# OpenNLPLab/ACR_WSSS

Measured on AMD Instinct MI355X. Metric: img/s ACR-ViT-hybrid-base 448x448 train step, higher is better.
Workload: dtype f32_split; 1 GPU; BASELINE configs[1]: ViT-hybrid-base (DPT) 448x448, batch 16 per GPU, ACR train step (2 views, fwd+bwd+SGD); global_batch=16, classes=20, alpha=125, parallelism=dp1

## Files before the change

### acr_wsss_amd/csrc/attn_f32.h

```cpp
#pragma once
#include <hip/hip_runtime.h>
#include <stdint.h>

struct AttnGeom {
    int B, H, T;
    float scale;
    int64_t sb, st, sh;
    int64_t osb, ost, osh;
};

void acr_attn_fwd_f32_dma(const AttnGeom& g, const float* q, const float* k, const float* v, float* o, float* lse2, float* pmean,
                          int64_t pmean_sb, int64_t pmean_st, hipStream_t st);
void acr_attn_bwd_f32_dma(const AttnGeom& g, const float* q, const float* k, const float* v, const float* o, const float* d_o,
                          const float* lse2, const float* gm, int64_t gm_sb, int64_t gm_st, float* dq, float* dk, float* dv,
                          float* delta, hipStream_t st);

void acr_attn_fwd_f32_sres(const AttnGeom& g, const float* q, const float* k, const float* v, float* o, float* lse2, float* scores,
                           float* pmean, int64_t pmean_sb, int64_t pmean_st, hipStream_t st);
void acr_attn_bwd_f32_sres(const AttnGeom& g, const float* q, const float* k, const float* v, const float* o, const float* d_o,
                           const float* lse2, const float* scores, const float* gm, int64_t gm_sb, int64_t gm_st, float* dq,
                           float* dk, float* dv, float* delta, hipStream_t st);
void acr_attn_pmean_sres(const AttnGeom& g, const float* scores, const float* lse2, float* pmean, int64_t pmean_sb, int64_t pmean_st,
                         hipStream_t st);
void acr_attn_delta_sres(const AttnGeom& g, const float* scores, const float* o, const float* d_o, const float* lse2, const float* gm,
                         int64_t gm_sb, int64_t gm_st, float* delta, hipStream_t st);

int64_t acr_attn_x3_scores_floats(const AttnGeom& g);
int64_t acr_attn_x3_bwd_ws_floats(const AttnGeom& g);
bool acr_attn_x3_fwd_uses_split_tail(int T);
void acr_attn_fwd_f32_x3(const AttnGeom& g, const float* q, const float* k, const float* v, float* o, float* lse2, float* scores,
                         float* pmean, int64_t pmean_sb, int64_t pmean_st, hipStream_t st, char* oimg = nullptr);
void acr_attn_bwd_f32_x3(const AttnGeom& g, const float* q, const float* k, const float* v, const float* o, const float* d_o,
                         const float* lse2, const float* scores, const float* gm, int64_t gm_sb, int64_t gm_st, float* dq, float* dk,
                         float* dv, float* delta_ws, hipStream_t st);
```

### acr_wsss_amd/csrc/attn_f32_sres.hip

```cpp
#include <type_traits>

#include "acr_common.h"
#include "attn_f32.h"
#include "attn_f32_tiles.h"
#include "attn_f32_scores.h"
#include "attn_f32_sres_tails.h"


template <int NW>
__global__ __launch_bounds__(64 * NW, NW == 4 ? 2 : 1) void attn_fwd_sres_kernel(AttnGeom g, const float* __restrict__ q, const float* __restrict__ k,
                                                               const float* __restrict__ v, float* __restrict__ o,
                                                               float* __restrict__ lse2, float* __restrict__ sres, int ntail) {
    __shared__ __attribute__((aligned(1024))) float smem[4 * DT_FLOATS];
    __shared__ float mlsh[4 * 64];
    const int nmain = (int)gridDim.x - ntail;
    if (NW == 4 && (int)blockIdx.x >= nmain) {
        attn_fwd_tail_body<4>(smem, mlsh, g, q, k, v, o, lse2, sres, acr_xcd_remap((int)blockIdx.x - nmain, ntail));
        return;
    }
    const int NB = (g.T + 31) >> 5, nqt = ntail ? NB / NW : (NB + NW - 1) / NW;
    int id = acr_xcd_remap(blockIdx.x, nmain);
    const int qt = id % nqt; id /= nqt;
    const int hd = id % g.H;
    const int b = id / g.H;
// ... 38 lines not shown
        ATTN_SOFTMAX_STEP(s, m, l, o0, o1, p);
        __builtin_amdgcn_s_setprio(0);
        accop_x<VOFF, 0, false>(o0, p, lb);
        accop_x<VOFF, 1, false>(o1, p, lb);
    };
    for (int k0 = 0; k0 < g.T; k0 += 64) {
        step(k0, std::integral_constant<int, 0>{});
        if (k0 + 32 < g.T) step(k0 + 32, std::integral_constant<int, 1>{});
    }
    if (live && q0 + r < g.T) {
        const float inv = 1.f / l;
        ATTN_FWD_FINISH(g, o, lse2, b, hd, q0, r, h, o0, o1, m, l, inv);
    }
}

#ifndef DELTA4_MINB
#define DELTA4_MINB 1
#endif
template <int NW> __global__ __launch_bounds__(64 * NW, DELTA4_MINB) void attn_delta_sres4_kernel(AttnGeom g, int NB, const float* __restrict__ sres,
                                                               const float* __restrict__ o, const float* __restrict__ d_o,
                                                               const float* __restrict__ lse2, const float* __restrict__ gm,
                                                               int64_t gm_sb, int64_t gm_st, float* __restrict__ delta) {
    __shared__ __attribute__((aligned(16))) float gt[3][32 * 36];
    const int tid = threadIdx.x, lane = tid & 63, wave = tid >> 6;
    const int theta = lane & 31, hh = lane >> 5;
    const int HG = g.H / NW;
    const int hd = (blockIdx.x % HG) * NW + wave;
    const int t = blockIdx.x / HG;
    const int qb = t % NB, b = t / NB;
    const int qrow = qb * 32 + theta;
    const bool qok = qrow < g.T;
    const int qc = min(qrow, g.T - 1);
    float part = 0.f;
    {
        const int64_t off = (int64_t)b * g.osb + (int64_t)hd * g.osh + (int64_t)qc * g.ost + 32 * hh;
        const float* op = o + off;
        const float* dp = d_o + off;
#pragma unroll
        for (int i = 0; i < 8; ++i) {
            const f32x4 a = *reinterpret_cast<const f32x4*>(op + 4 * i), c = *reinterpret_cast<const f32x4*>(dp + 4 * i);
            part += a[0] * c[0] + a[1] * c[1] + a[2] * c[2] + a[3] * c[3];
        }
    }
    part += __shfl_xor(part, 32);
    const float l2q = qok ? lse2[((int64_t)b * g.H + hd) * g.T + qrow] : INFINITY;
    const float* sp = sres + attn_score_block(g.H, NB, b, hd, qb, 0) + lane * 4;
    const bool loader = tid < 256;
    const int lrow = (tid & 255) >> 3, lc = (tid & 7) * 4;
    const float* gl = gm + (int64_t)b * gm_sb + (int64_t)min(qb * 32 + lrow, g.T - 1) * gm_st + lc;
    const int nfull = g.T >> 5;
    float rho = 0.f;
    f32x4 sv[3][4], gn[3];
    auto fetch = [&](int kb, int set) {
        if (loader) gn[set] = *reinterpret_cast<const f32x4*>(gl + kb * 32);
#pragma unroll
        for (int gq = 0; gq < 4; ++gq) sv[set][gq] = SRES_LOAD_NT(sp + (int64_t)kb * SB_FLOATS + gq * 256);
// ... 89 lines not shown
        float* ob = out + (int64_t)b * out_sb;
        if (key < g.T) {
#pragma unroll
            for (int i = 0; i < 16; ++i) {
                const int row = 2 * i + hh;
                const int qq = qb * 32 + row;
                if (qq < g.T) ob[(int64_t)qq * out_st + key] = tl[row * 33 + theta];
            }
        }
    }
}

__global__ __launch_bounds__(256) void attn_delta_sres_kernel(AttnGeom g, int NB, const float* __restrict__ sres,
                                                              const float* __restrict__ o, const float* __restrict__ d_o,
                                                              const float* __restrict__ lse2, const float* __restrict__ gm,
                                                              int64_t gm_sb, int64_t gm_st, float* __restrict__ delta) {
    const int tid = threadIdx.x, lane = tid & 63, wave = tid >> 6;
    const int theta = lane & 31, hh = lane >> 5;
    int id = blockIdx.x * 4 + wave;
    if (id >= g.B * NB * g.H) return;
    const int hd = id % g.H;
    const int t = id / g.H;
    const int qb = t % NB, b = t / NB;
    const int qrow = qb * 32 + theta;
    const bool qok = qrow < g.T;
    const int qc = min(qrow, g.T - 1);
    float part = 0.f;
    {
        const int64_t off = (int64_t)b * g.osb + (int64_t)hd * g.osh + (int64_t)qc * g.ost + 32 * hh;
        const float* op = o + off;
        const float* dp = d_o + off;
#pragma unroll
        for (int i = 0; i < 8; ++i) {
            const f32x4 a = *reinterpret_cast<const f32x4*>(op + 4 * i), c = *reinterpret_cast<const f32x4*>(dp + 4 * i);
            part += a[0] * c[0] + a[1] * c[1] + a[2] * c[2] + a[3] * c[3];
        }
    }
    part += __shfl_xor(part, 32);
    float rho = 0.f;
    if (gm != nullptr) {
        const float l2q = qok ? lse2[((int64_t)b * g.H + hd) * g.T + qrow] : INFINITY;
        const float* sp = sres + attn_score_block(g.H, NB, b, hd, qb, 0) + lane * 4;
        const float* gr = gm + (int64_t)b * gm_sb + (int64_t)qc * gm_st;
        const int nfull = g.T >> 5;
#pragma unroll 4
        for (int kb = 0; kb < nfull; ++kb) {
            f32x4 sv[4], gv[4];
#pragma unroll
            for (int gq = 0; gq < 4; ++gq) {
                sv[gq] = SRES_LOAD(sp + (int64_t)kb * SB_FLOATS + gq * 256);
// ... 233 lines not shown
    const int NB = (g.T + 31) / 32;
    const int ntail = attn_split_tail(NB, 4) ? g.B * g.H : 0;
    const int nmain = g.B * g.H * (ntail ? NB / 4 : (NB + 3) / 4);
    hipLaunchKernelGGL(attn_fwd_sres_kernel<4>, dim3(nmain + ntail), dim3(256), 0, st, g, q, k, v, o, lse2, scores, ntail);
    if (pmean) acr_attn_pmean_sres(g, scores, lse2, pmean, pmean_sb, pmean_st, st);
}

void acr_attn_pmean_sres(const AttnGeom& g, const float* scores, const float* lse2, float* pmean, int64_t pmean_sb, int64_t pmean_st,
                         hipStream_t st) {
    const int NB = (g.T + 31) / 32;
    hipLaunchKernelGGL(attn_pmean_sres_kernel, dim3((g.B * NB * NB + 3) / 4), dim3(256), 0, st, g, NB, scores, lse2, pmean, pmean_sb,
                       pmean_st);
}

void acr_attn_delta_sres(const AttnGeom& g, const float* scores, const float* o, const float* d_o, const float* lse2, const float* gm,
                         int64_t gm_sb, int64_t gm_st, float* delta, hipStream_t st) {
    const int NB = (g.T + 31) / 32;
#ifndef DELTA4_NW
#define DELTA4_NW 4
#endif
    if (gm != nullptr && (g.H % DELTA4_NW) == 0 && acr_opt(ACR_OPT_ATTN_DELTA_1HEAD) == 0)
        hipLaunchKernelGGL(attn_delta_sres4_kernel<DELTA4_NW>, dim3(g.B * NB * (g.H / DELTA4_NW)), dim3(64 * DELTA4_NW), 0, st, g, NB, scores, o, d_o,
                           lse2, gm, gm_sb, gm_st, delta);
    else
        hipLaunchKernelGGL(attn_delta_sres_kernel, dim3((g.B * NB * g.H + 3) / 4), dim3(256), 0, st, g, NB, scores, o, d_o, lse2, gm, gm_sb,
                           gm_st, delta);
}

void acr_attn_bwd_f32_sres(const AttnGeom& g, const float* q, const float* k, const float* v, const float* o, const float* d_o,
                           const float* lse2, const float* scores, const float* gm, int64_t gm_sb, int64_t gm_st, float* dq,
                           float* dk, float* dv, float* delta, hipStream_t st) {
    const int nt = (g.T + 127) / 128, NB = (g.T + 31) / 32;
    acr_attn_delta_sres(g, scores, o, d_o, lse2, gm, gm_sb, gm_st, delta, st);
    const int ntail = attn_split_tail(NB, 4) ? g.B * g.H : 0;
    const int nmain = g.B * g.H * (ntail ? NB / 4 : nt);
    hipLaunchKernelGGL(attn_bwd_sres_kernel, dim3(2 * nmain + 2 * ntail), dim3(256), 0, st, g, q, k, v, d_o, lse2, (const float*)delta,
                       scores, gm, gm_sb, gm_st, dq, dk, dv, ntail);
}
```

### acr_wsss_amd/csrc/attn_f32_x3.hip

```cpp
#include <type_traits>

#include "acr_split.h"
#include "attn_f32.h"
#include "attn_f32_scores.h"
#include "attn_f32_sres_tails.h"

typedef __bf16 bf16_t;

#define X3_PLANE_B (32 * 64 * 2)
#define X3_TILE_B (3 * X3_PLANE_B)
#define X3_SLOT_B (2 * X3_TILE_B)


__device__ __forceinline__ void x3_wait_vm(int n) { attn_wait_vm<false, 9, 8, 7, 5, 4, 1>(n); }
__device__ __forceinline__ void x3_barrier(int n_younger) {
    x3_wait_vm(n_younger);
    acr_barrier_nofence();
}

struct X3Geom {
    int B, H, T, D;
    float scale;
    int64_t plane;
    int64_t osb, ost, osh;
// ... 528 lines not shown
    const int64_t n8 = (int64_t)g.B * g.T * g.H * 8;
    hipLaunchKernelGGL(x3_split_kernel, dim3((unsigned)((n8 + 255) / 256), 3), dim3(256), 0, st, a);
    const int NB = (g.T + 31) / 32;
    const int ntail = (acr_attn_x3_fwd_uses_split_tail(g.T) && oimg == nullptr) ? g.B * g.H : 0;
    hipLaunchKernelGGL(attn_fwd_x3_kernel, dim3(g.B * g.H * (ntail ? NB / 4 : (NB + 3) / 4) + ntail), dim3(256), 0, st, x, (const bf16_t*)planes,
                       (const bf16_t*)(planes + 3 * x.plane), (const bf16_t*)(planes + 6 * x.plane), o, lse2, scores, q, k, v, g, ntail, oimg);
    if (pmean) acr_attn_pmean_sres(g, scores, lse2, pmean, pmean_sb, pmean_st, st);
}

void acr_attn_bwd_f32_x3(const AttnGeom& g, const float* q, const float* k, const float* v, const float* o, const float* d_o,
                         const float* lse2, const float* scores, const float* gm, int64_t gm_sb, int64_t gm_st, float* dq, float* dk,
                         float* dv, float* delta_ws, hipStream_t st) {
    const X3Geom x = x3_geom(g);
    const bf16_t* planes = reinterpret_cast<const bf16_t*>(scores + attn_score_floats(g.B, g.H, g.T));
    bf16_t* dop = reinterpret_cast<bf16_t*>(delta_ws + (((int64_t)g.B * g.H * g.T + 3) & ~(int64_t)3));
    X3SplitArgs a;
    a.src[0] = d_o; a.src[1] = a.src[2] = nullptr;
    a.sb = g.osb; a.st = g.ost; a.sh = g.osh; a.dst = dop; a.plane = x.plane; a.B = g.B; a.T = g.T; a.H = g.H;
    const int64_t n8 = (int64_t)g.B * g.T * g.H * 8;
    hipLaunchKernelGGL(x3_split_kernel, dim3((unsigned)((n8 + 255) / 256), 1), dim3(256), 0, st, a);
    acr_attn_delta_sres(g, scores, o, d_o, lse2, gm, gm_sb, gm_st, delta_ws, st);
    const int NB = (g.T + 31) / 32;
    const int ntail = attn_split_tail(NB, X3_BW) ? g.B * g.H : 0;
    const int nmain = g.B * g.H * (ntail ? NB / X3_BW : (NB + X3_BW - 1) / X3_BW);
    hipLaunchKernelGGL(attn_bwd_x3_kernel, dim3(2 * nmain + 2 * ntail), dim3(64 * X3_BW), 0, st, x, planes, planes + 3 * x.plane,
                       planes + 6 * x.plane, (const bf16_t*)dop, lse2, (const float*)delta_ws, scores, gm, gm_sb, gm_st, dq, dk, dv, q, k, v, d_o, g,
                       ntail);
}

extern "C" int acr_split3_bf16(const float* x, int64_t rows, int64_t cols, int64_t ld, void* planes, int64_t plane_stride, void* stream) {
    ACR_CHECK_ARG(x && planes, "acr_split3_bf16: null pointer");
    ACR_CHECK_ARG(rows > 0 && cols > 0 && (cols % 8) == 0 && (ld % 4) == 0 && ld >= cols, "acr_split3_bf16: need cols %% 8 == 0, ld %% 4 == 0, ld >= cols");
    ACR_CHECK_ARG(plane_stride >= rows * cols && (plane_stride % 8) == 0, "acr_split3_bf16: plane stride must cover rows * cols and be a multiple of 8");
    ACR_CHECK_ARG(((uintptr_t)x & 15) == 0 && ((uintptr_t)planes & 15) == 0, "acr_split3_bf16: 16-byte alignment");
    const int64_t n = rows * (cols >> 3);
    ACR_CHECK_ARG((n + 255) / 256 < (1ll << 31), "acr_split3_bf16: too large");
// ... 5 lines not shown
```

### acr_wsss_amd/csrc/layernorm.hip

```cpp
#include "acr_reduce.h"
#include "acr_split.h"

typedef __bf16 bf16_t;
#define LN_MAXV 4
#define LN_WAVES 4

template <int NV, typename T>
__global__ __launch_bounds__(256) void ln_fwd_kernel(const T* __restrict__ x, const T* __restrict__ gamma,
                                                     const T* __restrict__ beta, T* __restrict__ y,
                                                     float* __restrict__ stats, int M, int C, float eps) {
    const int lane = threadIdx.x & 63;
    const int gw = blockIdx.x * LN_WAVES + (threadIdx.x >> 6), nw = gridDim.x * LN_WAVES;
    const float inv_c = 1.f / (float)C;
    f32x4 ga[NV], be[NV];
#pragma unroll
    for (int i = 0; i < NV; ++i) {
        ga[i] = acr_load4<T>(gamma + (i * 64 + lane) * 4);
        be[i] = acr_load4<T>(beta + (i * 64 + lane) * 4);
    }
    for (int row = gw; row < M; row += nw) {
        const T* xr = x + (int64_t)row * C;
        f32x4 xv[NV];
        float s = 0.f;
#pragma unroll
// ... 63 lines not shown
            acr_store4<T>(dx + (int64_t)row * C + (i * 64 + lane) * 4, o);
        }
    }
    __shared__ float sh[LN_WAVES][2 * 256 * LN_MAXV];
    const int wv = threadIdx.x >> 6;
#pragma unroll
    for (int i = 0; i < NV; ++i) {
        *reinterpret_cast<f32x4*>(&sh[wv][(i * 64 + lane) * 4]) = dg[i];
        *reinterpret_cast<f32x4*>(&sh[wv][C + (i * 64 + lane) * 4]) = db[i];
    }
    __syncthreads();
    float* pg = part + (int64_t)blockIdx.x * 2 * C;
    for (int c = threadIdx.x; c < 2 * C; c += 256) pg[c] = (sh[0][c] + sh[1][c]) + (sh[2][c] + sh[3][c]);
}

template <typename T>
__global__ __launch_bounds__(256) void ln_param_reduce_kernel(const float* __restrict__ part, int np, int C,
                                                              T* __restrict__ dgamma, T* __restrict__ dbeta) {
    __shared__ float sh[8][32];
    const int cl = threadIdx.x & 31, grp = threadIdx.x >> 5;
    const int c = blockIdx.x * 32 + cl;
    float s = 0.f;
    const int per = (np + 7) / 8, w0 = grp * per, w1 = min(w0 + per, np);
    int w = w0;
    for (; w + 8 <= w1; w += 8) {
        float t[8];
#pragma unroll
        for (int u = 0; u < 8; ++u) t[u] = part[(int64_t)(w + u) * 2 * C + c];
#pragma unroll
        for (int u = 0; u < 8; ++u) s += t[u];
    }
    for (; w < w1; ++w) s += part[(int64_t)w * 2 * C + c];
    sh[grp][cl] = s;
    __syncthreads();
    if (grp == 0) {
        float tot = 0.f;
#pragma unroll
        for (int u = 0; u < 8; ++u) tot += sh[u][cl];
        if (c < C) acr_store1<T>(dgamma + c, tot); else acr_store1<T>(dbeta + c - C, tot);
    }
}

static int ln_grid(int M) {
    int g = (M + LN_WAVES - 1) / LN_WAVES;
    return g < 1024 ? g : 1024;
}
extern "C" size_t acr_layernorm_ws_floats(int32_t M, int32_t C) { return (size_t)ln_grid(M) * 2 * (size_t)C; }

static int ln_check(const char* who, int M, int C) {
    ACR_CHECK_ARG(M > 0 && C > 0 && (C % 256) == 0 && C <= 256 * LN_MAXV, "%s: C=%d must be a multiple of 256 and <= 1024", who, C);
    return ACR_OK;
}
#define LN_DISPATCH(KERNEL, TT, ...)                                                                  \
    switch (C / 256) {                                                                                 \
// ... 114 lines not shown
    ACR_CHECK_ARG(ln_al16(x) && ln_al16(gamma) && ln_al16(beta) && ln_al16(image), "acr_layernorm_image_f32: x / gamma / beta / image must be 16-byte aligned");
    const int nkb = C / IMG_BK;
    const dim3 grid((unsigned)(((M + IMG_ROWS - 1) / IMG_ROWS) * (IMG_ROWS / 32)));
    hipStream_t st = (hipStream_t)stream;
    char* img = reinterpret_cast<char*>(image);
#define LNI(NC) case NC: hipLaunchKernelGGL(ln_image_kernel<NC>, grid, dim3(256), 0, st, x, gamma, beta, img, stats, M, nkb, eps); break;
    switch (C / 64) {
        LNI(4) LNI(8) LNI(12) LNI(16)
        default:
            acr_set_error("acr_layernorm_image_f32: C = %d not instantiated (256, 512, 768, 1024: what acr_layernorm_bwd_f32 takes)", C);
            return ACR_ERR_UNSUPPORTED;
    }
#undef LNI
    return acr_check_launch("acr_layernorm_image_f32");
}
```

### acr_wsss_amd/ops.py

```python
import os
import numpy as np
import torch
from torch.autograd import Function

from . import _abi
from . import _lib as L

HEAD_DIM = 64
ATTN_F32_SCORES = True


def pad4(n):
    return (n + 3) & ~3


def _desc(B, H, T, dtype, packed_qkv=True, math=0):
    D = H * HEAD_DIM
    d = L.AttnDesc()
    d.B, d.H, d.T, d.head_dim = B, H, T, HEAD_DIM
    d.dtype = L.ACR_F32_BF16X3 if (math == 1 and dtype == torch.float32) else L.dtype_code(dtype)
    d.scale = HEAD_DIM ** -0.5
    d.qkv_sb, d.qkv_st, d.qkv_sh = T * 3 * D, 3 * D, HEAD_DIM
    d.o_sb, d.o_st, d.o_sh = T * D, D, HEAD_DIM
    return d
# ... 569 lines not shown
    ws = torch.empty(nws, dtype=torch.float32, device=dev) if nws else None
    tok = _t0("gemm_x3_" + mode, M, N, K)
    L.check(lib.acr_gemm_x3(md, act, L.ptr(a_img), L.ptr(b_img), L.ptr(bias), L.ptr(aux), aux.stride(0) if aux is not None else 0, L.ptr(c),
                            c.stride(0) if c is not None else N, L.ptr(c2), L.ptr(colsum), M, N, K, L.ptr(ws), L.stream_ptr()), "acr_gemm_x3")
    _t1(tok)
    return c


X3_IMAGE_EPILOGUES = True


def x3_image_empty(rows, cols, device):
    return torch.empty(L.load().acr_x3_image_floats(rows, cols), dtype=torch.float32, device=device)


def _f32_ok(*ts):
    return all(t is None or (t.dtype == torch.float32 and t.is_cuda and t.stride(-1) == 1 and (t.dim() == 1 or t.stride(0) % 4 == 0)
                             and t.data_ptr() % 16 == 0) for t in ts)


def linear_f32_usable(x, weight):
    K = x.shape[-1]
    N = weight.shape[0]
    return (x.is_cuda and x.dtype == torch.float32 and weight.dtype == torch.float32 and x.is_contiguous()
            and weight.is_contiguous() and K % 4 == 0 and N % 4 == 0 and K >= 32 and N >= 32 and x.numel() // K >= 1
            and _al16(x, weight))


class LinearF32Fn(Function):

# ... 19 lines not shown
            gemm_f32_raw("nt", x2, weight, y, bias=bias, aux=r2, math=math)
            ctx.save_for_backward(x2, weight)
        ctx.has_bias, ctx.has_resid, ctx.owner = bias is not None, resid is not None, owner
        return y.reshape(*shp[:-1], N)

    @staticmethod
    def backward(ctx, dy):
        x2, weight = ctx.saved_tensors
        N, K = weight.shape
        dy2 = dy.reshape(-1, N)
        if not dy2.is_contiguous():
            dy2 = dy2.contiguous()
        dx = dw = db = None
        want_db = ctx.has_bias and ctx.needs_input_grad[2]
        if ctx.images:
            if not _f32_ok(dy2):
                dy2 = dy2.clone()
            xi = x2
            db = torch.empty(N, dtype=torch.float32, device=dy.device) if want_db else None
            dyi = x3_image(dy2, colsum=db)
            if ctx.needs_input_grad[0]:
                dx = torch.empty((ctx.M, K), dtype=torch.float32, device=dy.device)
                gemm_x3("nt", dyi, weight_image(weight, ctx.owner, True), dx, N)
                dx = dx.reshape(*dy.shape[:-1], K)
            if ctx.needs_input_grad[1]:
                dw = torch.empty((N, K), dtype=torch.float32, device=dy.device)
                gemm_x3("tn", dyi, xi, dw, ctx.M)
            return dx, dw, db, (dy if ctx.has_resid else None), None, None, None
        if ctx.needs_input_grad[0]:
            dx = torch.empty((dy2.shape[0], K), dtype=torch.float32, device=dy.device)
            _dx_f32(dy2, weight, ctx.owner, dx, math=ctx.math)
            dx = dx.reshape(*dy.shape[:-1], K)
        if ctx.needs_input_grad[1]:
            dw = torch.empty((N, K), dtype=torch.float32, device=dy.device)
            db = torch.empty(N, dtype=torch.float32, device=dy.device) if want_db else None
# ... 40 lines not shown
        ctx.save_for_backward(x2, h, a, w1, w2)
        return y.reshape(*shp[:-1], D)

    @staticmethod
    def backward(ctx, dy):
        x2, h, a, w1, w2 = ctx.saved_tensors
        need = ctx.needs_input_grad
        dy2 = dy.reshape(-1, dy.shape[-1])
        if not dy2.is_contiguous():
            dy2 = dy2.contiguous()
        M, Hd = h.shape
        dev = dy.device
        math = ctx.math
        dw1 = db1 = dw2 = db2 = dx = None
        if ctx.images:
            if not _f32_ok(dy2):
                dy2 = dy2.clone()
            xi, ai = x2, a
            D = w2.shape[0]
            db2 = torch.empty(D, dtype=torch.float32, device=dev) if need[4] else None
            dyi = x3_image(dy2, colsum=db2)
            if need[3]:
                dw2 = torch.empty_like(w2)
                gemm_x3("tn", dyi, ai, dw2, M)
            db1 = torch.empty(Hd, dtype=torch.float32, device=dev) if need[2] else None
            if ctx.epi:
                dhi = x3_image_empty(M, Hd, dev)
                gemm_x3("nt", dyi, weight_image(w2, ctx.fc2, True), None, D, aux=h, act=4, c2=dhi, colsum=db1, shape=(M, Hd))
            else:
                dh = torch.empty_like(h)
                gemm_x3("nt", dyi, weight_image(w2, ctx.fc2, True), dh, D, aux=h, act=2)
                dhi = x3_image(dh, colsum=db1)
            if need[1]:
                dw1 = torch.empty_like(w1)
                gemm_x3("tn", dhi, xi, dw1, M)
            if need[0]:
# ... 16 lines not shown
        elif need[2]:
            db1 = dh.sum(0)
        if need[0]:
            dx = torch.empty_like(x2)
            _dx_f32(dh, w1, ctx.fc1, dx, math=math)
            dx = dx.reshape(*dy.shape[:-1], w1.shape[1])
        return dx, dw1, db1, dw2, db2, (dy if ctx.has_resid else None), None, None, None, None


def mlp_f32_usable(x, fc1, fc2, resid=None):
    return (linear_f32_usable(x, fc1.weight) and fc2.weight.dtype == torch.float32 and fc1.bias is not None
            and fc2.bias is not None and fc2.weight.is_contiguous() and fc2.weight.shape[0] % 4 == 0
            and _al16(fc2.weight, fc1.bias, fc2.bias, resid))


def mlp_f32(x, fc1, fc2, resid=None, math=0, x_image=None):
    return MlpF32Fn.apply(x, fc1.weight, fc1.bias, fc2.weight, fc2.bias, resid, fc1, fc2, math, x_image)


def linear_or_hip(x, lin, resid=None, use_hip=True, math=0, x_image=None):
    if x_image is not None:
        return LinearF32Fn.apply(x, lin.weight, lin.bias, resid, lin, math, x_image)
    if (use_hip and x.is_cuda and x.dtype == torch.bfloat16 and lin.weight.dtype == torch.bfloat16
            and lin.weight.shape[1] % 64 == 0 and x.is_contiguous() and _al16(x, lin.weight)):
        return LinearBf16Fn.apply(x, lin.weight, lin.bias, resid, lin)
    if (use_hip and linear_f32_usable(x, lin.weight) and not torch.is_autocast_enabled()
            and (math != 2 or _al16(lin.bias, resid))):
        return LinearF32Fn.apply(x, lin.weight, lin.bias, resid, lin, math)
    y = torch.nn.functional.linear(x, lin.weight, lin.bias)
    return y if resid is None else resid + y


class MaxPoolSameFn(Function):

    @staticmethod
    def forward(ctx, x, pt, pl, ph, pw):
        x = x.contiguous()
# ... 343 lines not shown
def conv_s2(x, weight, imgs=None):
    return ConvS2Fn.apply(x, weight, imgs)


def conv1x1(x, weight, wt=None, math=0, imgs=None):
    return Conv1x1Fn.apply(x, weight, wt, math, imgs)[0]


def conv1x1_skip(x, weight, wt=None, math=0, imgs=None):
    return Conv1x1Fn.apply(x, weight, wt, math, imgs)


class LayerNormFn(Function):

    @staticmethod
    def forward(ctx, x, weight, bias, eps, image=False):
        C = x.shape[-1]
        x2 = x.reshape(-1, C)
        M = x2.shape[0]
        lib = L.load()
        stats = torch.empty(2 * M, dtype=torch.float32, device=x.device)
        ctx.save_for_backward(x2, weight, stats)
        ctx.set_materialize_grads(False)
        if image:
            img = x3_image_empty(M, C, x.device)
            L.check(lib.acr_layernorm_image_f32(L.ptr(x2), L.ptr(weight), L.ptr(bias), L.ptr(img), L.ptr(stats), M, C, eps, L.stream_ptr()),
                    "acr_layernorm_image_f32")
            ctx.mark_non_differentiable(img)
            return x.new_empty(1).expand(x.shape), x.view_as(x), img
        y = torch.empty_like(x2)
        fwd = lib.acr_layernorm_fwd_f32 if x.dtype == torch.float32 else lib.acr_layernorm_fwd_bf16
        L.check(fwd(L.ptr(x2), L.ptr(weight), L.ptr(bias), L.ptr(y), L.ptr(stats), M, C, eps, L.stream_ptr()), "acr_layernorm_fwd")
        return y.reshape(x.shape), x.view_as(x)

    @staticmethod
    def backward(ctx, dy, dskip, dimg=None):
        x2, weight, stats = ctx.saved_tensors
        M, C = x2.shape
        if dy is None:
            return dskip, None, None, None, None
        lib = L.load()
        dy2 = dy.reshape(M, C)
        if not dy2.is_contiguous() or dy2.dtype != x2.dtype:
            dy2 = dy2.to(x2.dtype).contiguous()
        ds2 = None
        if dskip is not None:
            ds2 = dskip.reshape(M, C)
            if not ds2.is_contiguous() or ds2.dtype != x2.dtype:
                ds2 = ds2.to(x2.dtype).contiguous()
        dx = torch.empty_like(x2)
        ws = torch.empty(lib.acr_layernorm_ws_floats(M, C), dtype=torch.float32, device=x2.device)
        dg = torch.empty(C, dtype=x2.dtype, device=x2.device)
        db = torch.empty(C, dtype=x2.dtype, device=x2.device)
        bwd = lib.acr_layernorm_bwd_f32 if x2.dtype == torch.float32 else lib.acr_layernorm_bwd_bf16
        L.check(bwd(L.ptr(dy2), L.ptr(x2), L.ptr(weight), L.ptr(stats), L.ptr(ds2), L.ptr(dx), L.ptr(ws), L.ptr(dg), L.ptr(db), M, C,
                    L.stream_ptr()), "acr_layernorm_bwd")
        return dx.reshape(dy.shape), dg, db, None, None


def layer_norm_fusable(x, ln):
    C = x.shape[-1]
    return (x.is_cuda and x.dtype in (torch.bfloat16, torch.float32) and ln.weight.dtype == x.dtype and x.is_contiguous()
            and C % 256 == 0 and C <= 1024 and not (x.dtype == torch.float32 and torch.is_autocast_enabled())
            and _al16(x, ln.weight, ln.bias))


def layer_norm(x, ln):
    if layer_norm_fusable(x, ln):
        return LayerNormFn.apply(x, ln.weight, ln.bias, ln.eps, False)[0]
    return torch.nn.functional.layer_norm(x, (x.shape[-1],), ln.weight, ln.bias, ln.eps)


def layer_norm_skip(x, ln):
    if layer_norm_fusable(x, ln):
        return LayerNormFn.apply(x, ln.weight, ln.bias, ln.eps, False)
    return torch.nn.functional.layer_norm(x, (x.shape[-1],), ln.weight, ln.bias, ln.eps), x


class TokensFn(Function):

    @staticmethod
    def forward(ctx, y, bias, prefix, pos):
        B, D = y.shape[:2]
        T = y.shape[2] * y.shape[3]
        P = prefix.shape[0]
        tok = torch.empty((B, P + T, D), dtype=torch.float32, device=y.device)
        L.check(L.load().acr_tokens_fwd_f32(L.ptr(y), L.ptr(bias), L.ptr(prefix), L.ptr(pos), L.ptr(tok), B, D, T, P, L.stream_ptr()), "acr_tokens_fwd_f32")
        ctx.geom = (tuple(y.shape), P)
        return tok

# ... 15 lines not shown


def tokens(y, bias, prefix, pos):
    return TokensFn.apply(y, bias, prefix, pos)


def ln_image_usable(x, ln, lin, math):
    C = x.shape[-1]
    return (math == 1 and X3_IMAGES and x.is_cuda and x.dtype == torch.float32
            and x.is_contiguous() and ln.weight.dtype == torch.float32 and ln.bias is not None and C % 256 == 0 and C <= 1024
            and not torch.is_autocast_enabled() and lin.weight.dtype == torch.float32 and lin.weight.is_contiguous() and lin.weight.shape[1] == C
            and lin.weight.shape[0] % 4 == 0 and lin.weight.shape[0] >= 32 and _f32_ok(x, ln.weight, ln.bias, lin.weight, lin.bias))


def layer_norm_image(x, ln):
    return LayerNormFn.apply(x, ln.weight, ln.bias, ln.eps, True)


GN_ACT = {"none": 0, "relu": 1, "add_relu": 2}


def groupnorm_fusable(x, resid=None):
    if not (x.is_cuda and x.dtype in (torch.bfloat16, torch.float32) and x.dim() == 4 and x.is_contiguous() and _al16(x, resid)):
        return False
    N, C, H, W = x.shape
    if x.dtype == torch.float32:
        if C % 32 or C // 32 > 32 or (H * W) % 4 or torch.is_autocast_enabled():
            return False
    elif C % 32 or C // 32 > 64 or (H * W) % 8 or (C // 32) * H * W // 8 > 1024 * 13:
        return False
    return resid is None or (resid.shape == x.shape and resid.dtype == x.dtype and resid.is_contiguous())
# ... 233 lines not shown
```

### include/acr_hip.h

```cpp
#ifndef ACR_HIP_H
#define ACR_HIP_H

#include <stddef.h>
#include <stdint.h>

#ifdef __cplusplus
extern "C" {
#endif

#define ACR_ABI_VERSION 2

typedef enum acr_status {
    ACR_OK = 0,
    ACR_ERR_INVALID = -1,
    ACR_ERR_LAUNCH = -2,
    ACR_ERR_UNSUPPORTED = -3
} acr_status;

typedef enum acr_dtype { ACR_F32 = 0, ACR_BF16 = 1, ACR_BF16_F32MATH = 2, ACR_F32_BF16X3 = 3 } acr_dtype;

typedef enum acr_math { ACR_MATH_F32 = 0, ACR_MATH_BF16X3 = 1, ACR_MATH_FP16X2 = 2 } acr_math;
#define ACR_FP16X2_REL 2.384185791015625e-07
#define ACR_FP16X2_FLOOR 1.8189894035458565e-12

// ... 163 lines not shown
int acr_transpose_many_bf16(const void* table, const int32_t* blk_tensor, int32_t nblocks, void* stream);
int acr_transpose_many_f32(const void* table, const int32_t* blk_tensor, int32_t nblocks, void* stream);

size_t acr_layernorm_ws_floats(int32_t M, int32_t C);
int acr_layernorm_fwd_bf16(const void* x, const void* gamma, const void* beta, void* y, float* stats, int32_t M,
                           int32_t C, float eps, void* stream);
int acr_layernorm_bwd_bf16(const void* dy, const void* x, const void* gamma, const float* stats, const void* dskip,
                           void* dx, float* ws, void* dgamma, void* dbeta, int32_t M, int32_t C, void* stream);

int acr_layernorm_fwd_f32(const float* x, const float* gamma, const float* beta, float* y, float* stats, int32_t M, int32_t C,
                          float eps, void* stream);
int acr_layernorm_bwd_f32(const float* dy, const float* x, const float* gamma, const float* stats, const float* dskip, float* dx,
                          float* ws, float* dgamma, float* dbeta, int32_t M, int32_t C, void* stream);
int acr_layernorm_image_f32(const float* x, const float* gamma, const float* beta, float* image, float* stats, int32_t M, int32_t C, float eps,
                            void* stream);

int acr_tokens_fwd_f32(const float* y, const float* bias, const float* prefix, const float* pos, float* tok, int32_t B, int32_t D, int32_t T,
                       int32_t P, void* stream);
int acr_tokens_bwd_f32(const float* dtok, float* dy, float* dpos, int32_t B, int32_t D, int32_t T, int32_t P, void* stream);

int acr_groupnorm_fwd_bf16(const void* x, const void* resid, const void* gamma, const void* beta, void* y,
                           float* stats, int32_t N, int32_t C, int32_t HW, float eps, int32_t act, void* stream);
int acr_groupnorm_bwd_bf16(const void* dy, const void* x, const void* resid, const void* gamma, const void* beta,
                           const float* stats, void* dx, void* dresid, float* dgamma_part, float* dbeta_part,
                           void* dgamma, void* dbeta, int32_t N, int32_t C, int32_t HW, int32_t act, void* stream);

size_t acr_groupnorm_fwd_ws_floats(int32_t N, int32_t C, int32_t HW);
int acr_groupnorm_fwd_f32(const float* x, const float* resid, const float* gamma, const float* beta, float* y, float* stats,
                          int32_t N, int32_t C, int32_t HW, float eps, int32_t act, float* ws, void* stream);
int acr_groupnorm_bwd_f32(const float* dy, const float* x, const float* resid, const float* gamma, const float* beta,
// ... 171 lines not shown
```

Baseline: 128.7 img/s.

## Fuse bf16x3 split of gradients into layernorm backward and attention delta kernels

The layernorm backward gains an image variant that writes dx along with its three-plane bf16 split image and column sum. It parks these so the following linear or MLP backward can reuse them instead of launching a separate x3_image split pass. Separately, the attention delta kernel now writes the bf16x3 planes of d_o directly, removing a standalone split kernel launch and an extra read of d_o. The cost is extra registers and stores in the fused kernels, plus Python-side bookkeeping that matches parked tensors by storage pointer and version.

```diff
diff --git a/acr_wsss_amd/csrc/attn_f32.h b/acr_wsss_amd/csrc/attn_f32.h
--- a/acr_wsss_amd/csrc/attn_f32.h
+++ b/acr_wsss_amd/csrc/attn_f32.h
@@ -23,7 +23,7 @@
 void acr_attn_pmean_sres(const AttnGeom& g, const float* scores, const float* lse2, float* pmean, int64_t pmean_sb, int64_t pmean_st,
                          hipStream_t st);
 void acr_attn_delta_sres(const AttnGeom& g, const float* scores, const float* o, const float* d_o, const float* lse2, const float* gm,
-                         int64_t gm_sb, int64_t gm_st, float* delta, hipStream_t st);
+                         int64_t gm_sb, int64_t gm_st, float* delta, hipStream_t st, void* do_planes = nullptr);
 
 int64_t acr_attn_x3_scores_floats(const AttnGeom& g);
 int64_t acr_attn_x3_bwd_ws_floats(const AttnGeom& g);
diff --git a/acr_wsss_amd/csrc/attn_f32_sres.hip b/acr_wsss_amd/csrc/attn_f32_sres.hip
--- a/acr_wsss_amd/csrc/attn_f32_sres.hip
+++ b/acr_wsss_amd/csrc/attn_f32_sres.hip
@@ -1,6 +1,7 @@
 #include <type_traits>
 
 #include "acr_common.h"
+#include "acr_split.h"
 #include "attn_f32.h"
 #include "attn_f32_tiles.h"
 #include "attn_f32_scores.h"
@@ -76,13 +77,22 @@
     }
 }
 
+__device__ __forceinline__ void delta_do_planes(__bf16* dst, int64_t dplane, const f32x4& lo, const f32x4& hi) {
+    bf16x8 p0, p1, p2;
+    split3_bf16(lo, hi, p0, p1, p2);
+    *reinterpret_cast<bf16x8*>(dst) = p0;
+    *reinterpret_cast<bf16x8*>(dst + dplane) = p1;
+    *reinterpret_cast<bf16x8*>(dst + 2 * dplane) = p2;
+}
+
 #ifndef DELTA4_MINB
 #define DELTA4_MINB 1
 #endif
 template <int NW> __global__ __launch_bounds__(64 * NW, DELTA4_MINB) void attn_delta_sres4_kernel(AttnGeom g, int NB, const float* __restrict__ sres,
                                                                const float* __restrict__ o, const float* __restrict__ d_o,
                                                                const float* __restrict__ lse2, const float* __restrict__ gm,
-                                                               int64_t gm_sb, int64_t gm_st, float* __restrict__ delta) {
+                                                               int64_t gm_sb, int64_t gm_st, float* __restrict__ delta,
+                                                               __bf16* __restrict__ dop, int64_t dplane) {
     __shared__ __attribute__((aligned(16))) float gt[3][32 * 36];
     const int tid = threadIdx.x, lane = tid & 63, wave = tid >> 6;
     const int theta = lane & 31, hh = lane >> 5;
@@ -98,10 +108,14 @@
         const int64_t off = (int64_t)b * g.osb + (int64_t)hd * g.osh + (int64_t)qc * g.ost + 32 * hh;
         const float* op = o + off;
         const float* dp = d_o + off;
-#pragma unroll
-        for (int i = 0; i < 8; ++i) {
+        __bf16* pl = (dop && qok) ? dop + ((int64_t)b * g.T + qrow) * (g.H * 64) + hd * 64 + 32 * hh : nullptr;
+#pragma unroll
+        for (int i = 0; i < 8; i += 2) {
             const f32x4 a = *reinterpret_cast<const f32x4*>(op + 4 * i), c = *reinterpret_cast<const f32x4*>(dp + 4 * i);
             part += a[0] * c[0] + a[1] * c[1] + a[2] * c[2] + a[3] * c[3];
+            const f32x4 a1 = *reinterpret_cast<const f32x4*>(op + 4 * i + 4), c1 = *reinterpret_cast<const f32x4*>(dp + 4 * i + 4);
+            part += a1[0] * c1[0] + a1[1] * c1[1] + a1[2] * c1[2] + a1[3] * c1[3];
+            if (pl) delta_do_planes(pl + 4 * i, dplane, c, c1);
         }
     }
     part += __shfl_xor(part, 32);
@@ -221,7 +235,8 @@
 __global__ __launch_bounds__(256) void attn_delta_sres_kernel(AttnGeom g, int NB, const float* __restrict__ sres,
                                                               const float* __restrict__ o, const float* __restrict__ d_o,
                                                               const float* __restrict__ lse2, const float* __restrict__ gm,
-                                                              int64_t gm_sb, int64_t gm_st, float* __restrict__ delta) {
+                                                              int64_t gm_sb, int64_t gm_st, float* __restrict__ delta,
+                                                               __bf16* __restrict__ dop, int64_t dplane) {
     const int tid = threadIdx.x, lane = tid & 63, wave = tid >> 6;
     const int theta = lane & 31, hh = lane >> 5;
     int id = blockIdx.x * 4 + wave;
@@ -237,10 +252,14 @@
         const int64_t off = (int64_t)b * g.osb + (int64_t)hd * g.osh + (int64_t)qc * g.ost + 32 * hh;
         const float* op = o + off;
         const float* dp = d_o + off;
-#pragma unroll
-        for (int i = 0; i < 8; ++i) {
+        __bf16* pl = (dop && qok) ? dop + ((int64_t)b * g.T + qrow) * (g.H * 64) + hd * 64 + 32 * hh : nullptr;
+#pragma unroll
+        for (int i = 0; i < 8; i += 2) {
             const f32x4 a = *reinterpret_cast<const f32x4*>(op + 4 * i), c = *reinterpret_cast<const f32x4*>(dp + 4 * i);
             part += a[0] * c[0] + a[1] * c[1] + a[2] * c[2] + a[3] * c[3];
+            const f32x4 a1 = *reinterpret_cast<const f32x4*>(op + 4 * i + 4), c1 = *reinterpret_cast<const f32x4*>(dp + 4 * i + 4);
+            part += a1[0] * c1[0] + a1[1] * c1[1] + a1[2] * c1[2] + a1[3] * c1[3];
+            if (pl) delta_do_planes(pl + 4 * i, dplane, c, c1);
         }
     }
     part += __shfl_xor(part, 32);
@@ -504,17 +523,19 @@
 }
 
 void acr_attn_delta_sres(const AttnGeom& g, const float* scores, const float* o, const float* d_o, const float* lse2, const float* gm,
-                         int64_t gm_sb, int64_t gm_st, float* delta, hipStream_t st) {
+                         int64_t gm_sb, int64_t gm_st, float* delta, hipStream_t st, void* do_planes) {
     const int NB = (g.T + 31) / 32;
+    __bf16* dop = reinterpret_cast<__bf16*>(do_planes);
+    const int64_t dplane = (int64_t)g.B * g.T * g.H * 64;
 #ifndef DELTA4_NW
 #define DELTA4_NW 4
 #endif
     if (gm != nullptr && (g.H % DELTA4_NW) == 0 && acr_opt(ACR_OPT_ATTN_DELTA_1HEAD) == 0)
         hipLaunchKernelGGL(attn_delta_sres4_kernel<DELTA4_NW>, dim3(g.B * NB * (g.H / DELTA4_NW)), dim3(64 * DELTA4_NW), 0, st, g, NB, scores, o, d_o,
-                           lse2, gm, gm_sb, gm_st, delta);
+                           lse2, gm, gm_sb, gm_st, delta, dop, dplane);
     else
         hipLaunchKernelGGL(attn_delta_sres_kernel, dim3((g.B * NB * g.H + 3) / 4), dim3(256), 0, st, g, NB, scores, o, d_o, lse2, gm, gm_sb,
-                           gm_st, delta);
+                           gm_st, delta, dop, dplane);
 }
 
 void acr_attn_bwd_f32_sres(const AttnGeom& g, const float* q, const float* k, const float* v, const float* o, const float* d_o,
diff --git a/acr_wsss_amd/csrc/attn_f32_x3.hip b/acr_wsss_amd/csrc/attn_f32_x3.hip
--- a/acr_wsss_amd/csrc/attn_f32_x3.hip
+++ b/acr_wsss_amd/csrc/attn_f32_x3.hip
@@ -566,12 +566,7 @@
     const X3Geom x = x3_geom(g);
     const bf16_t* planes = reinterpret_cast<const bf16_t*>(scores + attn_score_floats(g.B, g.H, g.T));
     bf16_t* dop = reinterpret_cast<bf16_t*>(delta_ws + (((int64_t)g.B * g.H * g.T + 3) & ~(int64_t)3));
-    X3SplitArgs a;
-    a.src[0] = d_o; a.src[1] = a.src[2] = nullptr;
-    a.sb = g.osb; a.st = g.ost; a.sh = g.osh; a.dst = dop; a.plane = x.plane; a.B = g.B; a.T = g.T; a.H = g.H;
-    const int64_t n8 = (int64_t)g.B * g.T * g.H * 8;
-    hipLaunchKernelGGL(x3_split_kernel, dim3((unsigned)((n8 + 255) / 256), 1), dim3(256), 0, st, a);
-    acr_attn_delta_sres(g, scores, o, d_o, lse2, gm, gm_sb, gm_st, delta_ws, st);
+    acr_attn_delta_sres(g, scores, o, d_o, lse2, gm, gm_sb, gm_st, delta_ws, st, dop);
     const int NB = (g.T + 31) / 32;
     const int ntail = attn_split_tail(NB, X3_BW) ? g.B * g.H : 0;
     const int nmain = g.B * g.H * (ntail ? NB / X3_BW : (NB + X3_BW - 1) / X3_BW);
diff --git a/acr_wsss_amd/csrc/layernorm.hip b/acr_wsss_amd/csrc/layernorm.hip
--- a/acr_wsss_amd/csrc/layernorm.hip
+++ b/acr_wsss_amd/csrc/layernorm.hip
@@ -101,9 +101,9 @@
     for (int c = threadIdx.x; c < 2 * C; c += 256) pg[c] = (sh[0][c] + sh[1][c]) + (sh[2][c] + sh[3][c]);
 }
 
-template <typename T>
+template <typename T, int NVEC = 2>
 __global__ __launch_bounds__(256) void ln_param_reduce_kernel(const float* __restrict__ part, int np, int C,
-                                                              T* __restrict__ dgamma, T* __restrict__ dbeta) {
+                                                              T* __restrict__ dgamma, T* __restrict__ dbeta, float* __restrict__ dcol = nullptr) {
     __shared__ float sh[8][32];
     const int cl = threadIdx.x & 31, grp = threadIdx.x >> 5;
     const int c = blockIdx.x * 32 + cl;
@@ -113,18 +113,20 @@
     for (; w + 8 <= w1; w += 8) {
         float t[8];
 #pragma unroll
-        for (int u = 0; u < 8; ++u) t[u] = part[(int64_t)(w + u) * 2 * C + c];
+        for (int u = 0; u < 8; ++u) t[u] = part[(int64_t)(w + u) * NVEC * C + c];
 #pragma unroll
         for (int u = 0; u < 8; ++u) s += t[u];
     }
-    for (; w < w1; ++w) s += part[(int64_t)w * 2 * C + c];
+    for (; w < w1; ++w) s += part[(int64_t)w * NVEC * C + c];
     sh[grp][cl] = s;
     __syncthreads();
     if (grp == 0) {
         float tot = 0.f;
 #pragma unroll
         for (int u = 0; u < 8; ++u) tot += sh[u][cl];
-        if (c < C) acr_store1<T>(dgamma + c, tot); else acr_store1<T>(dbeta + c - C, tot);
+        if (c < C) acr_store1<T>(dgamma + c, tot);
+        else if (NVEC == 2 || c < 2 * C) acr_store1<T>(dbeta + c - C, tot);
+        else dcol[c - 2 * C] = tot;
     }
 }
 
@@ -269,3 +271,124 @@
 #undef LNI
     return acr_check_launch("acr_layernorm_image_f32");
 }
+
+typedef int ln_i32x2 __attribute__((ext_vector_type(2)));
+typedef int ln_i32x4 __attribute__((ext_vector_type(4)));
+#define LN_STG_B 416
+template <int NV>
+__global__ __launch_bounds__(256, NV <= 3 ? 4 : 3) void ln_bwd_image_kernel(
+    const float* __restrict__ dy, const float* __restrict__ x, const float* __restrict__ gamma, const float* __restrict__ stats,
+    const float* __restrict__ dskip, float* __restrict__ dx, char* __restrict__ img, float* __restrict__ part, int M, int C) {
+    constexpr int nkb = NV * 16;
+    constexpr int STG = 2 * nkb * LN_STG_B, RED = LN_WAVES * 256 * NV * 4;
+    __shared__ __attribute__((aligned(16))) char smem[STG > RED ? STG : RED];
+    const int lane = threadIdx.x & 63, wv = threadIdx.x >> 6;
+    const int nw = gridDim.x * LN_WAVES;
+    const float inv_c = 1.f / (float)C;
+    f32x4 ga[NV], dg[NV], db[NV], dc[NV];
+#pragma unroll
+    for (int i = 0; i < NV; ++i) {
+        ga[i] = acr_load4<float>(gamma + (i * 64 + lane) * 4);
+        dg[i] = (f32x4){0.f, 0.f, 0.f, 0.f};
+        db[i] = (f32x4){0.f, 0.f, 0.f, 0.f};
+        dc[i] = (f32x4){0.f, 0.f, 0.f, 0.f};
+    }
+    int it = 0;
+    for (int base = blockIdx.x * LN_WAVES; base < M; base += nw, ++it) {
+        const int row = base + wv;
+        const bool live = row < M;
+        const int rt = row & 127;
+        const int half = (((lane >> 1) & 1) ^ IMG_ROW_SWZ(rt)) * 16 + (lane & 1) * 8;
+        char* stg = smem + (it & 1) * (nkb * LN_STG_B) + (lane >> 2) * LN_STG_B + wv * IMG_ROW_B + half;
+        if (live) {
+            const float mean = stats[2 * row], rstd = stats[2 * row + 1];
+            f32x4 xh[NV], g[NV];
+            float s1 = 0.f, s2 = 0.f;
+#pragma unroll
+            for (int i = 0; i < NV; ++i) {
+                const f32x4 xv = acr_load4<float>(x + (int64_t)row * C + (i * 64 + lane) * 4);
+                const f32x4 dv = acr_load4<float>(dy + (int64_t)row * C + (i * 64 + lane) * 4);
+#pragma unroll
+                for (int e = 0; e < 4; ++e) {
+                    xh[i][e] = (xv[e] - mean) * rstd;
+                    g[i][e] = dv[e] * ga[i][e];
+                    s1 += g[i][e];
+                    s2 = fmaf(g[i][e], xh[i][e], s2);
+                    dg[i][e] = fmaf(dv[e], xh[i][e], dg[i][e]);
+                    db[i][e] += dv[e];
+                }
+            }
+            const float c1 = acr_wave_sum(s1) * inv_c, c2 = acr_wave_sum(s2) * inv_c;
+#pragma unroll
+            for (int i = 0; i < NV; ++i) {
+                f32x4 o;
+#pragma unroll
+                for (int e = 0; e < 4; ++e) o[e] = rstd * (g[i][e] - c1 - xh[i][e] * c2);
+                if (dskip) o += acr_load4<float>(dskip + (int64_t)row * C + (i * 64 + lane) * 4);
+                acr_store4<float>(dx + (int64_t)row * C + (i * 64 + lane) * 4, o);
+                dc[i] += o;
+                bf16x4 p[3];
+#pragma unroll
+                for (int e = 0; e < 4; ++e) {
+                    __bf16 h0, h1, h2;
+                    split3_bf16(o[e], h0, h1, h2);
+                    p[0][e] = h0; p[1][e] = h1; p[2][e] = h2;
+                }
+#pragma unroll
+                for (int q = 0; q < 3; ++q) *reinterpret_cast<bf16x4*>(stg + i * 16 * LN_STG_B + q * (LN_WAVES * IMG_ROW_B)) = p[q];
+            }
+        } else {
+#pragma unroll
+            for (int i = 0; i < NV; ++i)
+#pragma unroll
+                for (int q = 0; q < 3; ++q) *reinterpret_cast<ln_i32x2*>(stg + i * 16 * LN_STG_B + q * (LN_WAVES * IMG_ROW_B)) = (ln_i32x2){0, 0};
+        }
+        __syncthreads();
+        const char* src = smem + (it & 1) * (nkb * LN_STG_B);
+        char* dst = img + IMG_STAGE_OFF(base >> 7, nkb, 0, 3) + (base & 127) * IMG_ROW_B;
+        for (int c = threadIdx.x; c < nkb * 24; c += 256) {
+            const int kb = c / 24, rem = c - kb * 24;
+            *reinterpret_cast<ln_i32x4*>(dst + (int64_t)kb * (3 * IMG_PLANE_B) + (rem >> 3) * IMG_PLANE_B + (rem & 7) * 16) =
+                *reinterpret_cast<const ln_i32x4*>(src + kb * LN_STG_B + rem * 16);
+        }
+    }
+    const int gw = blockIdx.x * LN_WAVES + wv, m0 = (M + LN_WAVES - 1) & ~(LN_WAVES - 1);
+    for (int row = m0 + gw; row < ((M + IMG_ROWS - 1) & ~(IMG_ROWS - 1)); row += nw) {
+        char* chunk = img + IMG_STAGE_OFF(row >> 7, nkb, lane >> 2, 3) + planes_chunk_off(row & 127, (lane >> 1) & 1) + (lane & 1) * 8;
+#pragma unroll
+        for (int i = 0; i < NV; ++i)
+#pragma unroll
+            for (int q = 0; q < 3; ++q)
+                *reinterpret_cast<ln_i32x2*>(chunk + (int64_t)i * 16 * (3 * IMG_PLANE_B) + q * IMG_PLANE_B) = (ln_i32x2){0, 0};
+    }
+    float (*sh)[256 * NV] = reinterpret_cast<float (*)[256 * NV]>(smem);
+    float* pg = part + (int64_t)blockIdx.x * 3 * C;
+#pragma unroll
+    for (int v = 0; v < 3; ++v) {
+        __syncthreads();
+#pragma unroll
+        for (int i = 0; i < NV; ++i) *reinterpret_cast<f32x4*>(&sh[wv][(i * 64 + lane) * 4]) = v == 0 ? dg[i] : v == 1 ? db[i] : dc[i];
+        __syncthreads();
+        for (int c = threadIdx.x; c < C; c += 256) pg[v * C + c] = (sh[0][c] + sh[1][c]) + (sh[2][c] + sh[3][c]);
+    }
+}
+
+extern "C" size_t acr_layernorm_bwd_image_ws_floats(int32_t M, int32_t C) { return (size_t)ln_grid(M) * 3 * (size_t)C; }
+
+extern "C" int acr_layernorm_bwd_image_f32(const float* dy, const float* x, const float* gamma, const float* stats, const float* dskip,
+                                           float* dx, float* image, float* colsum, float* ws, float* dgamma, float* dbeta, int32_t M,
+                                           int32_t C, void* stream) {
+    ACR_CHECK_ARG(dy && x && gamma && stats && dx && image && colsum && ws && dgamma && dbeta, "acr_layernorm_bwd_image_f32: null pointer");
+    ACR_CHECK_ARG(ln_al16(dy) && ln_al16(x) && ln_al16(gamma) && ln_al16(dskip) && ln_al16(dx) && ln_al16(image),
+                  "acr_layernorm_bwd_image_f32: dy / x / gamma / dskip / dx / image must be 16-byte aligned (vector loads and stores)");
+    int rc = ln_check("acr_layernorm_bwd_image_f32", M, C);
+    if (rc) return rc;
+    const dim3 grid(ln_grid(M));
+    hipStream_t st = (hipStream_t)stream;
+    char* img = reinterpret_cast<char*>(image);
+#define LNBI(NV) case NV: hipLaunchKernelGGL((ln_bwd_image_kernel<NV>), grid, dim3(256), 0, st, dy, x, gamma, stats, dskip, dx, img, ws, M, C); break;
+    switch (C / 256) { LNBI(1) LNBI(2) LNBI(3) default: LNBI(4) }
+#undef LNBI
+    hipLaunchKernelGGL((ln_param_reduce_kernel<float, 3>), dim3(3 * C / 32), dim3(256), 0, st, (const float*)ws, ln_grid(M), C, dgamma, dbeta, colsum);
+    return acr_check_launch("acr_layernorm_bwd_image_f32");
+}
diff --git a/acr_wsss_amd/ops.py b/acr_wsss_amd/ops.py
--- a/acr_wsss_amd/ops.py
+++ b/acr_wsss_amd/ops.py
@@ -607,6 +607,46 @@
     return torch.empty(L.load().acr_x3_image_floats(rows, cols), dtype=torch.float32, device=device)
 
 
+DY_IMAGES = True
+DY_IMAGES_TAKEN = 0
+_DY_PARKED = []
+_DY_CLEANUP = [False]
+
+
+def _dy_images_clear():
+    del _DY_PARKED[:]
+    _DY_CLEANUP[0] = False
+
+
+def _park_dy_image(dx, img, colsum):
+    _DY_PARKED.append((dx, dx._version, img, colsum))
+    del _DY_PARKED[:-2]
+    if not _DY_CLEANUP[0]:
+        _DY_CLEANUP[0] = True
+        torch.autograd.Variable._execution_engine.queue_callback(_dy_images_clear)
+
+
+def _take_dy_image(dy2):
+    global DY_IMAGES_TAKEN
+    for i, (dx, ver, img, colsum) in enumerate(_DY_PARKED):
+        if (dy2.untyped_storage().data_ptr() == dx.untyped_storage().data_ptr() and dy2.storage_offset() == dx.storage_offset()
+                and dy2.shape == dx.shape and dy2.stride() == dx.stride() and dy2.dtype == dx.dtype and dy2._version == ver):
+            del _DY_PARKED[i]
+            DY_IMAGES_TAKEN += 1
+            return img, colsum
+    return None
+
+
+def _dy_image_or_pass(dy2, want_colsum):
+    got = _take_dy_image(dy2)
+    if got is not None:
+        return dy2, got[0], (got[1] if want_colsum else None)
+    if not _f32_ok(dy2):
+        dy2 = dy2.clone()
+    colsum = torch.empty(dy2.shape[1], dtype=torch.float32, device=dy2.device) if want_colsum else None
+    return dy2, x3_image(dy2, colsum=colsum), colsum
+
+
 def _f32_ok(*ts):
     return all(t is None or (t.dtype == torch.float32 and t.is_cuda and t.stride(-1) == 1 and (t.dim() == 1 or t.stride(0) % 4 == 0)
                              and t.data_ptr() % 16 == 0) for t in ts)
@@ -656,11 +696,8 @@
         dx = dw = db = None
         want_db = ctx.has_bias and ctx.needs_input_grad[2]
         if ctx.images:
-            if not _f32_ok(dy2):
-                dy2 = dy2.clone()
             xi = x2
-            db = torch.empty(N, dtype=torch.float32, device=dy.device) if want_db else None
-            dyi = x3_image(dy2, colsum=db)
+            dy2, dyi, db = _dy_image_or_pass(dy2, want_db)
             if ctx.needs_input_grad[0]:
                 dx = torch.empty((ctx.M, K), dtype=torch.float32, device=dy.device)
                 gemm_x3("nt", dyi, weight_image(weight, ctx.owner, True), dx, N)
@@ -731,12 +768,9 @@
         math = ctx.math
         dw1 = db1 = dw2 = db2 = dx = None
         if ctx.images:
-            if not _f32_ok(dy2):
-                dy2 = dy2.clone()
             xi, ai = x2, a
             D = w2.shape[0]
-            db2 = torch.empty(D, dtype=torch.float32, device=dev) if need[4] else None
-            dyi = x3_image(dy2, colsum=db2)
+            dy2, dyi, db2 = _dy_image_or_pass(dy2, need[4])
             if need[3]:
                 dw2 = torch.empty_like(w2)
                 gemm_x3("tn", dyi, ai, dw2, M)
@@ -783,13 +817,19 @@
             and _al16(fc2.weight, fc1.bias, fc2.bias, resid))
 
 
+def _tag_dy_image(y):
+    y._acr_dy_image = True
+    return y
+
+
 def mlp_f32(x, fc1, fc2, resid=None, math=0, x_image=None):
-    return MlpF32Fn.apply(x, fc1.weight, fc1.bias, fc2.weight, fc2.bias, resid, fc1, fc2, math, x_image)
+    y = MlpF32Fn.apply(x, fc1.weight, fc1.bias, fc2.weight, fc2.bias, resid, fc1, fc2, math, x_image)
+    return _tag_dy_image(y) if x_image is not None else y
 
 
 def linear_or_hip(x, lin, resid=None, use_hip=True, math=0, x_image=None):
     if x_image is not None:
-        return LinearF32Fn.apply(x, lin.weight, lin.bias, resid, lin, math, x_image)
+        return _tag_dy_image(LinearF32Fn.apply(x, lin.weight, lin.bias, resid, lin, math, x_image))
     if (use_hip and x.is_cuda and x.dtype == torch.bfloat16 and lin.weight.dtype == torch.bfloat16
             and lin.weight.shape[1] % 64 == 0 and x.is_contiguous() and _al16(x, lin.weight)):
         return LinearBf16Fn.apply(x, lin.weight, lin.bias, resid, lin)
@@ -1163,7 +1203,8 @@
 class LayerNormFn(Function):
 
     @staticmethod
-    def forward(ctx, x, weight, bias, eps, image=False):
+    def forward(ctx, x, weight, bias, eps, image=False, dy_image=False):
+        ctx.dy_image = image and dy_image
         C = x.shape[-1]
         x2 = x.reshape(-1, C)
         M = x2.shape[0]
@@ -1187,7 +1228,7 @@
         x2, weight, stats = ctx.saved_tensors
         M, C = x2.shape
         if dy is None:
-            return dskip, None, None, None, None
+            return dskip, None, None, None, None, None
         lib = L.load()
         dy2 = dy.reshape(M, C)
         if not dy2.is_contiguous() or dy2.dtype != x2.dtype:
@@ -1198,13 +1239,22 @@
             if not ds2.is_contiguous() or ds2.dtype != x2.dtype:
                 ds2 = ds2.to(x2.dtype).contiguous()
         dx = torch.empty_like(x2)
-        ws = torch.empty(lib.acr_layernorm_ws_floats(M, C), dtype=torch.float32, device=x2.device)
         dg = torch.empty(C, dtype=x2.dtype, device=x2.device)
         db = torch.empty(C, dtype=x2.dtype, device=x2.device)
+        if ctx.dy_image and DY_IMAGES and ctx.needs_input_grad[0] and _f32_ok(dy2, ds2):
+            img = x3_image_empty(M, C, x2.device)
+            colsum = torch.empty(C, dtype=torch.float32, device=x2.device)
+            ws = torch.empty(lib.acr_layernorm_bwd_image_ws_floats(M, C), dtype=torch.float32, device=x2.device)
+            L.check(lib.acr_layernorm_bwd_image_f32(L.ptr(dy2), L.ptr(x2), L.ptr(weight), L.ptr(stats), L.ptr(ds2), L.ptr(dx), L.ptr(img),
+                                                    L.ptr(colsum), L.ptr(ws), L.ptr(dg), L.ptr(db), M, C, L.stream_ptr()),
+                    "acr_layernorm_bwd_image_f32")
+            _park_dy_image(dx, img, colsum)
+            return dx.reshape(dy.shape), dg, db, None, None, None
+        ws = torch.empty(lib.acr_layernorm_ws_floats(M, C), dtype=torch.float32, device=x2.device)
         bwd = lib.acr_layernorm_bwd_f32 if x2.dtype == torch.float32 else lib.acr_layernorm_bwd_bf16
         L.check(bwd(L.ptr(dy2), L.ptr(x2), L.ptr(weight), L.ptr(stats), L.ptr(ds2), L.ptr(dx), L.ptr(ws), L.ptr(dg), L.ptr(db), M, C,
                     L.stream_ptr()), "acr_layernorm_bwd")
-        return dx.reshape(dy.shape), dg, db, None, None
+        return dx.reshape(dy.shape), dg, db, None, None, None
 
 
 def layer_norm_fusable(x, ln):
@@ -1216,13 +1266,13 @@
 
 def layer_norm(x, ln):
     if layer_norm_fusable(x, ln):
-        return LayerNormFn.apply(x, ln.weight, ln.bias, ln.eps, False)[0]
+        return LayerNormFn.apply(x, ln.weight, ln.bias, ln.eps, False, False)[0]
     return torch.nn.functional.layer_norm(x, (x.shape[-1],), ln.weight, ln.bias, ln.eps)
 
 
 def layer_norm_skip(x, ln):
     if layer_norm_fusable(x, ln):
-        return LayerNormFn.apply(x, ln.weight, ln.bias, ln.eps, False)
+        return LayerNormFn.apply(x, ln.weight, ln.bias, ln.eps, False, False)
     return torch.nn.functional.layer_norm(x, (x.shape[-1],), ln.weight, ln.bias, ln.eps), x
 
 
@@ -1268,7 +1318,7 @@
 
 
 def layer_norm_image(x, ln):
-    return LayerNormFn.apply(x, ln.weight, ln.bias, ln.eps, True)
+    return LayerNormFn.apply(x, ln.weight, ln.bias, ln.eps, True, getattr(x, "_acr_dy_image", False))
 
 
 GN_ACT = {"none": 0, "relu": 1, "add_relu": 2}
diff --git a/include/acr_hip.h b/include/acr_hip.h
--- a/include/acr_hip.h
+++ b/include/acr_hip.h
@@ -201,6 +201,9 @@
                           float* ws, float* dgamma, float* dbeta, int32_t M, int32_t C, void* stream);
 int acr_layernorm_image_f32(const float* x, const float* gamma, const float* beta, float* image, float* stats, int32_t M, int32_t C, float eps,
                             void* stream);
+size_t acr_layernorm_bwd_image_ws_floats(int32_t M, int32_t C);
+int acr_layernorm_bwd_image_f32(const float* dy, const float* x, const float* gamma, const float* stats, const float* dskip, float* dx,
+                                float* image, float* colsum, float* ws, float* dgamma, float* dbeta, int32_t M, int32_t C, void* stream);
 
 int acr_tokens_fwd_f32(const float* y, const float* bias, const float* prefix, const float* pos, float* tok, int32_t B, int32_t D, int32_t T,
                        int32_t P, void* stream);
```

New measurement: 128.5 img/s. About the same (-0.2%).
